# electronicarts/mesh2splat

Measured on AMD Instinct MI355X. Metric: Gaussians/sec emitted (mesh->3DGS conversion pass, density 1024^2), higher is better.
Workload: dtype f32

## Files before the change

mesh2splat_amd/csrc/m2s_devfn.h:

```cpp
#pragma once
#include "m2s_device.h"
#include "m2s_exact.h"

#pragma clang fp contract(off)

namespace m2s {

__device__ __forceinline__ float len3(float x, float y, float z) { return sqrtf((x * x + y * y) + z * z); }
__device__ __forceinline__ float len3sq(float x, float y, float z) { return (x * x + y * y) + z * z; }
__device__ __forceinline__ float inv_len3(float x, float y, float z) {
    const float q = len3sq(x, y, z);
    if (wave_all(in_sqrt_range(q))) return rcp_rn(sqrt_rn(q));
    return 1.0f / sqrtf(q);
}

__device__ __forceinline__ uint32_t wave_incl_scan(uint32_t v, int ) {
    v += (uint32_t)__builtin_amdgcn_update_dpp(0, (int)v, 0x111, 0xf, 0xf, true);
    v += (uint32_t)__builtin_amdgcn_update_dpp(0, (int)v, 0x112, 0xf, 0xf, true);
    v += (uint32_t)__builtin_amdgcn_update_dpp(0, (int)v, 0x114, 0xf, 0xf, true);
    v += (uint32_t)__builtin_amdgcn_update_dpp(0, (int)v, 0x118, 0xf, 0xf, true);
    v += (uint32_t)__builtin_amdgcn_update_dpp(0, (int)v, 0x142, 0xa, 0xf, true);
    v += (uint32_t)__builtin_amdgcn_update_dpp(0, (int)v, 0x143, 0xc, 0xf, true);
    return v;
}
// ... 515 lines not shown
    const uint32_t m = q[2u * (t0 >> 3)], end = q[2u * (t0 >> 3) + 1u];
    uniform = end > t_last;
    return m;
}

__device__ __forceinline__ bool setup_raster_for(const SceneDev& sc, uint32_t t, uint32_t mesh_hint, bool uniform_mesh,
                                                 uint32_t R, Raster& rs) {
    float p[9];
    load_positions(sc.tri, t, p);
    uint32_t m = uniform_mesh ? mesh_hint : find_mesh(sc, sc.tri_first + t);
    const MeshParams* mp = sc.meshes + m;
    Geo g;
    geo_setup(p, mp->bmin, mp->bmax, g);
    return raster_setup(g, R, rs);
}

constexpr float kUnorm8 = 0.003921568859368563f;

struct __attribute__((packed, aligned(4))) ComboPair { uint32_t v[6]; };

typedef const __attribute__((address_space(1))) char* GlobalBytes;
__device__ __forceinline__ GlobalBytes as_global(const void* p) { return (GlobalBytes)p; }
__device__ __forceinline__ ComboPair ld_combo(GlobalBytes base, uint32_t dword_off) {
    const __attribute__((address_space(1))) uint32_t* p = reinterpret_cast<const __attribute__((address_space(1))) uint32_t*>(base + (size_t)(dword_off * 4u));
    ComboPair r;
#pragma unroll
    for (int i = 0; i < 6; ++i) r.v[i] = p[i];
    return r;
}
__device__ __forceinline__ uint32_t ld_texel(GlobalBytes base, uint32_t texel) {
    return *reinterpret_cast<const __attribute__((address_space(1))) uint32_t*>(base + (size_t)(texel * 4u));
}


struct TriShade {
    int a1, b1, a2, b2;
    long long e1, e2;
    float inva, sx, sy, lod0;
    float4 rot;
    float lod1, lod2;
    uint32_t org;
    uint32_t mesh;
};
static_assert(sizeof(TriShade) == 80, "TriShade must be five float4");

struct TriShadeS {
    short a1, b1, a2, b2;
    int e1, e2;
    float inva, sx, sy, lod0;
    float4 rot;
    float lod1, lod2;
    uint32_t org;
    uint32_t mesh;
};
static_assert(sizeof(TriShadeS) == 64, "TriShadeS must be four float4");

__device__ __forceinline__ float lod_from_grad(float fw, float fh, float dudx, float dvdx, float dudy, float dvdy) {
    const float sx = dudx * fw, tx = dvdx * fh, sy = dudy * fw, ty = dvdy * fh;
    const float r2 = fmaxf(fma_(tx, tx, sx * sx), fma_(ty, ty, sy * sy));
    return 0.5f * fast_log2(r2);
}

template <class MP, class TS>
__device__ __forceinline__ void tri_shade_rest(const float p[9], const Geo& g, int a1, int b1, int a2, int b2, MP mp,
                                               float4 b0, float2 b1uv, TS& ts) {
    ts.mesh = 0;
    const float A1 = (float)a1 * 256.0f * ts.inva, B1 = (float)b1 * 256.0f * ts.inva;
    const float A2 = (float)a2 * 256.0f * ts.inva, B2 = (float)b2 * 256.0f * ts.inva;
    geo_flat(p, g, ts.sx, ts.sy, ts.rot);
    ts.lod0 = ts.lod1 = ts.lod2 = 0.0f;
    const auto ta = &mp->tex[0];
    const auto tn = &mp->tex[1];
    const auto tm = &mp->tex[2];
    const bool hasA = ta->texels != nullptr, hasN = tn->texels != nullptr, hasM = tm->texels != nullptr;
    if (hasA || hasN || hasM) {
        const float du1 = b0.z - b0.x, du2 = b1uv.x - b0.x, dv1 = b0.w - b0.y, dv2 = b1uv.y - b0.y;
        const float dudx = fma_(A2, du2, A1 * du1), dvdx = fma_(A2, dv2, A1 * dv1);
        const float dudy = fma_(B2, du2, B1 * du1), dvdy = fma_(B2, dv2, B1 * dv1);
        if (hasA) ts.lod0 = lod_from_grad((float)ta->w, (float)ta->h, dudx, dvdx, dudy, dvdy);
        if (hasN) ts.lod1 = (hasA && tn->w == ta->w && tn->h == ta->h) ? ts.lod0
                          : lod_from_grad((float)tn->w, (float)tn->h, dudx, dvdx, dudy, dvdy);
        if (hasM) ts.lod2 = (hasA && tm->w == ta->w && tm->h == ta->h) ? ts.lod0
                          : (hasN && tm->w == tn->w && tm->h == tn->h) ? ts.lod1
                          : lod_from_grad((float)tm->w, (float)tm->h, dudx, dvdx, dudy, dvdy);
        if (mp->combo.texels != nullptr) {
            const uint32_t nl = ta->n_levels;
            const float q = (float)(nl - 1), lambda = ts.lod0;
            float d = 0.0f, f = 0.0f;
            if (lambda > 0.0f) {
                if (lambda >= q) d = q;
                else { d = floorf(lambda); f = lambda - d; }
            }
            const uint32_t l0 = (uint32_t)d, l1 = min(l0 + 1u, nl - 1u);
            const uint32_t c1 = mp->combo.coff[1], c2 = mp->combo.coff[2], c3 = mp->combo.coff[3], c4 = mp->combo.coff[4];
            const uint32_t off0 = l0 == 0 ? 0u : l0 == 1 ? c1 : l0 == 2 ? c2 : l0 == 3 ? c3 : c4;
            const uint32_t off1 = l1 == 0 ? 0u : l1 == 1 ? c1 : l1 == 2 ? c2 : l1 == 3 ? c3 : c4;
            ts.lod0 = f;
            ts.lod1 = __uint_as_float(off0);
            ts.lod2 = __uint_as_float(off1);
            ts.mesh = (l0 | (l1 << 4)) << 24;
        }
    }
}

template <class MP>
__device__ __forceinline__ void tri_shade_setup(const float p[9], const Geo& g, const Raster& rs, MP mp,
                                                float4 b0, float2 b1, TriShade& ts) {
    {
#pragma clang fp contract(off)
        ts.inva = rcp_rn((float)rs.area2);
    }
    const long long Px0 = 256ll * rs.x0 + 128, Py0 = 256ll * rs.y0 + 128;
    ts.a1 = rs.a[1]; ts.b1 = rs.b[1]; ts.a2 = rs.a[2]; ts.b2 = rs.b[2];
    ts.e1 = (long long)rs.a[1] * Px0 + (long long)rs.b[1] * Py0 + rs.c[1];
    ts.e2 = (long long)rs.a[2] * Px0 + (long long)rs.b[2] * Py0 + rs.c[2];
    ts.org = ((uint32_t)rs.y0 << 12) | (uint32_t)rs.x0;
    tri_shade_rest(p, g, rs.a[1], rs.b[1], rs.a[2], rs.b[2], mp, b0, b1, ts);
}

template <class MP>
__device__ __forceinline__ void tri_shade_small(const float p[9], const Geo& g, const RasterHead& h, const RasterSmall& rs, MP mp, float4 b0, float2 b1,
                                                uint32_t m, TriShadeS& c) {
    {
#pragma clang fp contract(off)
        c.inva = rcp_rn((float)rs.area2);
    }
    c.a1 = (short)rs.a[1]; c.b1 = (short)rs.b[1]; c.a2 = (short)rs.a[2]; c.b2 = (short)rs.b[2];
    c.e1 = rs.e[1]; c.e2 = rs.e[2];
    c.org = ((uint32_t)h.y0 << 12) | (uint32_t)h.x0;
    tri_shade_rest(p, g, rs.a[1], rs.b[1], rs.a[2], rs.b[2], mp, b0, b1, c);
    c.mesh |= m;
}

struct TexTap {
    uint32_t o00, o10, o01, o11;
    float w00, w10, w01, w11;
};

__device__ __forceinline__ void tex_tap(uint32_t W, uint32_t H, uint32_t level_off, float uf, float vf, TexTap& t) {
    float up, vp;
    {
#pragma clang fp contract(off)
        up = uf * (float)W - 0.5f;
        vp = vf * (float)H - 0.5f;
    }
    const float fi = floorf(up), fj = floorf(vp);
    const float a = up - fi, b = vp - fj;
    int i0 = (int)fi, j0 = (int)fj;
    int i1 = i0 + 1, j1 = j0 + 1;
    i0 = i0 < 0 ? i0 + (int)W : i0;
    j0 = j0 < 0 ? j0 + (int)H : j0;
    i1 = i1 >= (int)W ? i1 - (int)W : i1;
    j1 = j1 >= (int)H ? j1 - (int)H : j1;
    const uint32_t r0 = level_off + __umul24((uint32_t)j0, W), r1 = level_off + __umul24((uint32_t)j1, W);
    t.o00 = r0 + (uint32_t)i0; t.o10 = r0 + (uint32_t)i1;
    t.o01 = r1 + (uint32_t)i0; t.o11 = r1 + (uint32_t)i1;
    const float na = 1.0f - a, nb = 1.0f - b;
    t.w00 = na * nb; t.w10 = a * nb; t.w01 = na * b; t.w11 = a * b;
}

struct TexState {
    TexTap lo, hi;
    float f;
};

template <class TD>
__device__ __forceinline__ void tex_state(TD t, float uf, float vf, float lambda, TexState& st) {
    const uint32_t nl = t->n_levels, w = t->w, h = t->h;
    const float q = (float)(nl - 1);
    float d = 0.0f, f = 0.0f;
    if (lambda > 0.0f) {
        if (lambda >= q) d = q;
        else { d = floorf(lambda); f = lambda - d; }
    }
    const uint32_t l0 = (uint32_t)d, l1 = min(l0 + 1u, nl - 1u);
    const uint32_t o1 = t->off[1], o2 = t->off[2], o3 = t->off[3], o4 = t->off[4];
    const uint32_t off0 = l0 == 0 ? 0u : l0 == 1 ? o1 : l0 == 2 ? o2 : l0 == 3 ? o3 : o4;
    const uint32_t off1 = l1 == 0 ? 0u : l1 == 1 ? o1 : l1 == 2 ? o2 : l1 == 3 ? o3 : o4;
    tex_tap(max(1u, w >> l0), max(1u, h >> l0), off0, uf, vf, st.lo);
    st.f = f;
    if (__ballot(f != 0.0f) != 0ull) tex_tap(max(1u, w >> l1), max(1u, h >> l1), off1, uf, vf, st.hi);
    else st.hi = st.lo;
}

struct TexFetch { uint32_t lo[4], hi[4]; };
__device__ __forceinline__ void tex_issue(const uint32_t* __restrict__ texels, const TexState& st, TexFetch& tf) {
    const GlobalBytes gb = as_global(texels);
    tf.lo[0] = ld_texel(gb, st.lo.o00); tf.lo[1] = ld_texel(gb, st.lo.o10); tf.lo[2] = ld_texel(gb, st.lo.o01); tf.lo[3] = ld_texel(gb, st.lo.o11);
    tf.hi[0] = ld_texel(gb, st.hi.o00); tf.hi[1] = ld_texel(gb, st.hi.o10); tf.hi[2] = ld_texel(gb, st.hi.o01); tf.hi[3] = ld_texel(gb, st.hi.o11);
}
template <int NCH>
__device__ __forceinline__ void tap_filter(const uint32_t t[4], const TexTap& tp, float out[NCH]) {
#pragma unroll
    for (int ch = 0; ch < NCH; ch++) {
        const float c00 = (float)((t[0] >> (8 * ch)) & 255u), c10 = (float)((t[1] >> (8 * ch)) & 255u);
        const float c01 = (float)((t[2] >> (8 * ch)) & 255u), c11 = (float)((t[3] >> (8 * ch)) & 255u);
        out[ch] = fma_(tp.w11, c11, fma_(tp.w01, c01, fma_(tp.w10, c10, tp.w00 * c00)));
    }
}
template <int NCH>
__device__ __forceinline__ void tex_finish(const TexFetch& tf, const TexState& st, float out[NCH]) {
    float lo[NCH], hi[NCH];
    tap_filter<NCH>(tf.lo, st.lo, lo);
    tap_filter<NCH>(tf.hi, st.hi, hi);
    const float f = st.f, nf = 1.0f - st.f;
#pragma unroll
    for (int ch = 0; ch < NCH; ch++) out[ch] = fma_(f, hi[ch], nf * lo[ch]) * kUnorm8;
}


struct ComboTap {
    uint32_t o0, o1;
    float w00, w10, w01, w11;
};

__device__ __forceinline__ void combo_tap(uint32_t level_off, uint32_t W, uint32_t H, float uf, float vf, ComboTap& t) {
    float up, vp;
    {
#pragma clang fp contract(off)
        up = uf * (float)W - 0.5f;
        vp = vf * (float)H - 0.5f;
    }
    const float fi = floorf(up), fj = floorf(vp);
    const float a = up - fi, b = vp - fj;
    int i0 = (int)fi, j0 = (int)fj;
    int j1 = j0 + 1;
    i0 = i0 < 0 ? i0 + (int)W : i0;
    j0 = j0 < 0 ? j0 + (int)H : j0;
    j1 = j1 >= (int)H ? j1 - (int)H : j1;
    const uint32_t stride = W + 1;
    t.o0 = level_off + (__umul24((uint32_t)j0, stride) + (uint32_t)i0) * 3u;
    t.o1 = level_off + (__umul24((uint32_t)j1, stride) + (uint32_t)i0) * 3u;
    const float na = 1.0f - a, nb = 1.0f - b;
    t.w00 = na * nb; t.w10 = a * nb; t.w01 = na * b; t.w11 = a * b;
}

__device__ __forceinline__ void combo_filter(const ComboPair& r0, const ComboPair& r1, const ComboTap& t, float out[9]) {
#define M2S_CH(word, sh) fma_(t.w11, (float)((r1.v[(word) + 3] >> (sh)) & 255u), fma_(t.w01, (float)((r1.v[word] >> (sh)) & 255u), \
                          fma_(t.w10, (float)((r0.v[(word) + 3] >> (sh)) & 255u), t.w00 * (float)((r0.v[word] >> (sh)) & 255u))))
    out[0] = M2S_CH(0, 0); out[1] = M2S_CH(0, 8); out[2] = M2S_CH(0, 16); out[3] = M2S_CH(0, 24);
    out[4] = M2S_CH(1, 0); out[5] = M2S_CH(1, 8); out[6] = M2S_CH(1, 16);
    out[7] = M2S_CH(2, 8); out[8] = M2S_CH(2, 16);
#undef M2S_CH
}

__device__ __forceinline__ float frac_repeat(float u) {
    float f = u - floorf(u);
    f = (f >= 0.0f) ? f : 0.0f;
    return fminf(f, 1.0f);
}

struct ComboFetch {
    ComboTap tlo, thi;
    ComboPair a0, a1, b0, b1;
    float f;
};
template <class MP, class TD, class TS>
__device__ __forceinline__ void combo_issue(MP mp, TD t, float uf, float vf, const TS& ts, ComboFetch& cf) {
    const uint32_t w = t->w, h = t->h;
    const float f = ts.lod0;
    const uint32_t off0 = __float_as_uint(ts.lod1), off1 = __float_as_uint(ts.lod2);
    const uint32_t l0 = (ts.mesh >> 24) & 15u, l1 = ts.mesh >> 28;
    const uint32_t* __restrict__ base = mp->combo.texels;
    ComboTap& tlo = cf.tlo;
    ComboTap& thi = cf.thi;
    cf.f = f;
    combo_tap(off0, max(1u, w >> l0), max(1u, h >> l0), uf, vf, tlo);
    combo_tap(off1, max(1u, w >> l1), max(1u, h >> l1), uf, vf, thi);
    const GlobalBytes gb = as_global(base);
    cf.a0 = ld_combo(gb, tlo.o0);
    cf.a1 = ld_combo(gb, tlo.o1);
    cf.b0 = ld_combo(gb, thi.o0);
    cf.b1 = ld_combo(gb, thi.o1);
#ifdef M2S_FUSED3_PRIO
    __builtin_amdgcn_s_setprio(0);
#endif
}
__device__ __forceinline__ void combo_finish(ComboFetch& cf, float out[9]) {
    ComboTap& tlo = cf.tlo;
    ComboTap& thi = cf.thi;
    const float f = cf.f;
    const float klo = (1.0f - f) * kUnorm8, khi = f * kUnorm8;
    tlo.w00 *= klo; tlo.w10 *= klo; tlo.w01 *= klo; tlo.w11 *= klo;
    thi.w00 *= khi; thi.w10 *= khi; thi.w01 *= khi; thi.w11 *= khi;
    float lo[9], hi[9];
    combo_filter(cf.a0, cf.a1, tlo, lo);
    combo_filter(cf.b0, cf.b1, thi, hi);
#pragma unroll
    for (int ch = 0; ch < 9; ch++) out[ch] = lo[ch] + hi[ch];
}
template <class MP, class TD, class TS>
__device__ __forceinline__ void combo_sample(MP mp, TD t, float uf, float vf, const TS& ts, float out[9]) {
    ComboFetch cf;
    combo_issue(mp, t, uf, vf, ts, cf);
    combo_finish(cf, out);
}


template <typename T>
__device__ __forceinline__ T ld_plane(const T* base, uint32_t t) {
    return *reinterpret_cast<const T*>(reinterpret_cast<const char*>(base) + (size_t)(t * (uint32_t)sizeof(T)));
}


template <class MP, class TS = TriShade, bool kComboOnly = false>
__device__ __forceinline__ void shade_from_tri(const TriPlanes& tp, uint32_t t, int x, int y, MP mp,
                                               const TS& ts, float4 rec[6], unsigned long long* stamps = nullptr,
                                               const float2* uvl = nullptr ) {
    const int dx256 = (x - (int)(ts.org & 0xFFFu)) * 256, dy256 = (y - (int)(ts.org >> 12)) * 256;
    float l1, l2;
    if constexpr (sizeof(ts.e1) == 4) {
        const int E1 = ts.e1 + (int)ts.a1 * dx256 + (int)ts.b1 * dy256;
        const int E2 = ts.e2 + (int)ts.a2 * dx256 + (int)ts.b2 * dy256;
        l1 = (float)E1 * ts.inva;
        l2 = (float)E2 * ts.inva;
    } else {
        const long long E1 = ts.e1 + (long long)ts.a1 * dx256 + (long long)ts.b1 * dy256;
        const long long E2 = ts.e2 + (long long)ts.a2 * dx256 + (long long)ts.b2 * dy256;
        l1 = i64_to_f32(E1) * ts.inva;
        l2 = i64_to_f32(E2) * ts.inva;
    }

    float4 b0 = make_float4(0, 0, 0, 0);
    float2 b1 = make_float2(0, 0);
    if (uvl == nullptr) {
        b0 = ld_plane(tp.B0, t);
        b1 = ld_plane(tp.B1, t);
    }
    const float4 a0 = ld_plane(tp.A0, t), a1 = ld_plane(tp.A1, t);
    const float a2 = ld_plane(tp.A2, t);
    const float4 c0 = ld_plane(tp.C0, t), c1 = ld_plane(tp.C1, t);
    const float c2 = ld_plane(tp.C2, t);
    const float4 d0 = ld_plane(tp.D0, t), d1 = ld_plane(tp.D1, t), d2 = ld_plane(tp.D2, t);
    float U, V;
    {
#pragma clang fp contract(off)
        if (uvl != nullptr) {
            const float2 q0 = uvl[0], q1 = uvl[1], q2 = uvl[2];
            U = (q0.x + l1 * q1.x) + l2 * q2.x;
            V = (q0.y + l1 * q1.y) + l2 * q2.y;
        } else {
            U = (b0.x + l1 * (b0.z - b0.x)) + l2 * (b1.x - b0.x);
            V = (b0.y + l1 * (b0.w - b0.y)) + l2 * (b1.y - b0.y);
        }
    }
#define M2S_LERP(f0, f1, f2) fma_(l2, (f2) - (f0), fma_(l1, (f1) - (f0), (f0)))

    const auto ta = &mp->tex[0];
    const auto tn = &mp->tex[1];
    const auto tm = &mp->tex[2];
    const uint32_t* xa = ta->texels;
    const uint32_t* xn = tn->texels;
    const uint32_t* xm = tm->texels;
    if (stamps) stamps[0] = __builtin_amdgcn_s_memtime();
    const float uf = frac_repeat(U), vf = frac_repeat(V);
    float col[4] = { 1.0f, 1.0f, 1.0f, 1.0f };
    float nrm[3] = { 0.0f, 0.0f, 1.0f };
    float metal = 0.1f, rough = 0.5f;
    const uint32_t* __restrict__ cmb = mp->combo.texels;
    if (cmb != nullptr) {
        float acc[9];
        combo_sample(mp, ta, uf, vf, ts, acc);
        col[0] = acc[0]; col[1] = acc[1]; col[2] = acc[2]; col[3] = acc[3];
        nrm[0] = acc[4]; nrm[1] = acc[5]; nrm[2] = acc[6];
        rough = acc[7]; metal = acc[8];
    } else if constexpr (!kComboOnly) {
        TexState sa, sn, sm;
        TexFetch fa, fn, fm;
        const bool n_like_a = xa != nullptr && xn != nullptr && tn->w == ta->w && tn->h == ta->h;
        const bool m_like_a = xa != nullptr && xm != nullptr && tm->w == ta->w && tm->h == ta->h;
        const bool m_like_n = xn != nullptr && xm != nullptr && tm->w == tn->w && tm->h == tn->h;
        if (xa != nullptr) tex_state(ta, uf, vf, ts.lod0, sa);
        if (xn != nullptr) { if (n_like_a) sn = sa; else tex_state(tn, uf, vf, ts.lod1, sn); }
        if (xm != nullptr) {
            if (xn != nullptr ? m_like_n : m_like_a) sm = (xn != nullptr) ? sn : sa;
            else tex_state(tm, uf, vf, ts.lod2, sm);
        }
        if (xa != nullptr) tex_issue(xa, sa, fa);
        if (xn != nullptr) tex_issue(xn, sn, fn);
        if (xm != nullptr) tex_issue(xm, sm, fm);
        if (xa != nullptr) tex_finish<4>(fa, sa, col);
        if (xn != nullptr) tex_finish<3>(fn, sn, nrm);
        if (xm != nullptr) {
            float sv[3];
            tex_finish<3>(fm, sm, sv);
            metal = sv[2]; rough = sv[1];
        }
    }
    if (stamps) stamps[1] = __builtin_amdgcn_s_memtime();
    const float Pxw = M2S_LERP(a0.x, a0.w, a1.z), Pyw = M2S_LERP(a0.y, a1.x, a1.w), Pzw = M2S_LERP(a0.z, a1.y, a2);
    const float Nx = M2S_LERP(c0.x, c0.w, c1.z), Ny = M2S_LERP(c0.y, c1.x, c1.w), Nz = M2S_LERP(c0.z, c1.y, c2);
    float ox = Nx, oy = Ny, oz = Nz;
    if (xn != nullptr) {
        const float Tx = M2S_LERP(d0.x, d1.x, d2.x), Ty = M2S_LERP(d0.y, d1.y, d2.y), Tz = M2S_LERP(d0.z, d1.z, d2.z);
        const float Tw = M2S_LERP(d0.w, d1.w, d2.w);
        float rx = fma_(nrm[0], 2.0f, -1.0f), ry = fma_(nrm[1], 2.0f, -1.0f), rz = fma_(nrm[2], 2.0f, -1.0f);
        float inv = fast_rsq(dot3_(rx, ry, rz, rx, ry, rz));
        rx *= inv; ry *= inv; rz *= inv;
        float bx = fma_(Ny, Tz, -(Nz * Ty)), by = fma_(Nz, Tx, -(Nx * Tz)), bz = fma_(Nx, Ty, -(Ny * Tx));
        inv = fast_rsq(dot3_(bx, by, bz, bx, by, bz)) * Tw;
        bx *= inv; by *= inv; bz *= inv;
        inv = fast_rsq(dot3_(Nx, Ny, Nz, Nx, Ny, Nz));
        const float nnx = Nx * inv, nny = Ny * inv, nnz = Nz * inv;
        const float wx = fma_(nnx, rz, fma_(bx, ry, Tx * rx)), wy = fma_(nny, rz, fma_(by, ry, Ty * rx)), wz = fma_(nnz, rz, fma_(bz, ry, Tz * rx));
        inv = fast_rsq(dot3_(wx, wy, wz, wx, wy, wz));
        ox = wx * inv; oy = wy * inv; oz = wz * inv;
    }
#undef M2S_LERP
    if (stamps) stamps[2] = __builtin_amdgcn_s_memtime();
    rec[0] = make_float4(Pxw, Pyw, Pzw, 1.0f);
    rec[1] = make_float4(col[0] * mp->color[0], col[1] * mp->color[1], col[2] * mp->color[2], col[3] * mp->color[3]);
    rec[2] = make_float4(ts.sx, ts.sy, 1e-7f, 0.0f);
    rec[3] = make_float4(ox, oy, oz, 0.0f);
    rec[4] = ts.rot;
    rec[5] = make_float4(metal, rough, 0.0f, 1.0f);
}

__device__ __forceinline__ void nt_store(float4* p, float4 v) {
    __builtin_nontemporal_store(v.x, &p->x); __builtin_nontemporal_store(v.y, &p->y);
    __builtin_nontemporal_store(v.z, &p->z); __builtin_nontemporal_store(v.w, &p->w);
}

}
```

mesh2splat_amd/csrc/m2s_fused3.hip:

```cpp
#include "m2s_fused_common.h"

#pragma clang fp contract(off)

namespace m2s {

#ifndef M2S_FUSED3_WAVES
#define M2S_FUSED3_WAVES 4
#endif
#ifndef M2S_FUSED3_ENTRIES
#define M2S_FUSED3_ENTRIES 1024
#endif
#ifndef M2S_FUSED3_STAGE
#define M2S_FUSED3_STAGE (M2S_FUSED3_WAVES >= 5 ? 16 : 32)
#endif
constexpr int kL3Team = 4;
constexpr int kL3Threads = kL3Team * 64;
constexpr uint32_t kL3Entries = (uint32_t)M2S_FUSED3_ENTRIES * kL3Team;
constexpr int kL3Stage = M2S_FUSED3_STAGE;
constexpr uint32_t kL3Wait = 1u << 24;
constexpr uint32_t kL3Stop = 1u << 28;

struct F3Ctl {
    unsigned long long base;
    unsigned long long total_w[kL3Team];
    uint32_t total_c[kL3Team];
    uint32_t counted[kL3Team];
    uint32_t expanded[kL3Team];
    uint32_t t0[kL3Team];
    uint32_t claimed;
    uint32_t base_state;
    uint32_t flags;
    uint32_t pad_;
};
struct F3Lds {
    float4 tri[kL3Team][64 * 4];
    uint32_t tskip[kL3Team][64];
    uint16_t entries[kL3Entries];
    float4 stage[kL3Team][kL3Stage * 6];
    F3Ctl ctl;
};
static_assert(sizeof(F3Lds) * M2S_FUSED3_WAVES <= 163840, "M2S_FUSED3_WAVES workgroups per CU must fit the 160 KB of LDS");
constexpr uint32_t kF3Irregular = 1u << 8;

__device__ __forceinline__ uint32_t l3_load(const uint32_t* p) { return __hip_atomic_load(p, __ATOMIC_ACQUIRE, __HIP_MEMORY_SCOPE_WORKGROUP); }
__device__ __forceinline__ void l3_store(uint32_t* p, uint32_t v) { __hip_atomic_store(p, v, __ATOMIC_RELEASE, __HIP_MEMORY_SCOPE_WORKGROUP); }
__device__ __forceinline__ uint32_t l3_uniform(const uint32_t* p) {
    return __builtin_amdgcn_readfirstlane(__hip_atomic_load(p, __ATOMIC_RELAXED, __HIP_MEMORY_SCOPE_WORKGROUP));
}
__device__ __forceinline__ void l3_fail(F3Ctl& C, uint32_t why, int lane) {
    if (lane == 0) {
        __hip_atomic_fetch_or(&C.flags, why, __ATOMIC_RELEASE, __HIP_MEMORY_SCOPE_WORKGROUP);
        __hip_atomic_fetch_add(&C.claimed, kL3Stop, __ATOMIC_RELAXED, __HIP_MEMORY_SCOPE_WORKGROUP);
    }
}

__device__ __forceinline__ bool f3_get_base(F3Ctl& C, unsigned long long* chain, uint32_t b0, int lane, uint32_t epoch, uint32_t* status,
                                            unsigned long long& base) {
    uint32_t st = l3_load(&C.base_state);
    if (st != 2) {
        uint32_t got = 1;
        if (lane == 0) {
            uint32_t expect = 0;
            got = __hip_atomic_compare_exchange_strong(&C.base_state, &expect, 1u, __ATOMIC_ACQ_REL, __ATOMIC_ACQUIRE, __HIP_MEMORY_SCOPE_WORKGROUP) ? 0u : 1u;
        }
        got = __builtin_amdgcn_readfirstlane(got);
        if (got == 0) {
            const unsigned long long b = b0 == 0 ? 0ull : lookback(chain, b0, lane, epoch, status);
            if (lane == 0) {
                C.base = b;
                chain_store(&chain[b0], kFlagPrefix | ((unsigned long long)epoch << kEpochShift) | ((b + C.total_w[0]) & kValMask));
            }
            l3_store(&C.base_state, 2u);
        } else {
            uint32_t spins = 0;
            while (l3_load(&C.base_state) != 2) {
                if (++spins > kL3Wait) { l3_fail(C, 1u, lane); return false; }
                __builtin_amdgcn_s_sleep(2);
            }
        }
    }
    base = C.base;
    return true;
}

#ifdef M2S_TIMELINE
__device__ unsigned long long g_tl_f3[16384 * 4 * 8];
#define TLF(k) do { __builtin_amdgcn_sched_barrier(0); if (lane == 0 && blockIdx.x < 16384u) g_tl_f3[((size_t)blockIdx.x * 4 + wave) * 8 + (k)] = wall_clock64(); __builtin_amdgcn_sched_barrier(0); } while (0)
#define TLFV(k, v) do { if (lane == 0 && blockIdx.x < 16384u) g_tl_f3[((size_t)blockIdx.x * 4 + wave) * 8 + (k)] = (v); } while (0)
#else
#define TLF(k) do { } while (0)
#define TLFV(k, v) do { } while (0)
#endif

__global__ void __launch_bounds__(kL3Threads, M2S_FUSED3_WAVES) k_fused3(SceneDev sc, uint32_t R, unsigned long long* __restrict__ chain,
                                                      unsigned long long limit, float4* __restrict__ out,
                                                      unsigned long long* __restrict__ total_out,
                                                      uint32_t* __restrict__ status , uint32_t epoch,
                                                      BigItem* __restrict__ biglist, uint32_t* __restrict__ bigmeta,
                                                      uint32_t tpw ,
                                                      RunInfo runs, BatchTable bt) {
    __shared__ F3Lds S;
    F3Ctl& C = S.ctl;
    const int lane = threadIdx.x & 63;
    const uint32_t wave = __builtin_amdgcn_readfirstlane(threadIdx.x >> 6);
    const uint32_t n_batches = bt.first ? bt.n : (sc.n_tri + tpw - 1u) / tpw;
    const uint32_t hb = blockIdx.x, xcd = hb & 7u, round = hb >> 3;
    const bool in_runs = runs.base != nullptr;
    const uint32_t rmask = (1u << runs.shift) - 1u;
    const unsigned long long etag = (unsigned long long)epoch << kEpochShift;
    uint32_t lb = hb;
    if (in_runs) {
        uint32_t rr = ((round >> runs.shift) << 3) + xcd;
        if (runs.order) rr = ((const __attribute__((address_space(4))) uint32_t*)runs.order)[rr];
        lb = (rr << runs.shift) + (round & rmask);
    }
    const bool band_first = in_runs && (round & rmask) == 0u;
    if (lb * (uint32_t)kL3Team >= n_batches) return;
    TLF(0);
    if (lane == 0) { C.counted[wave] = 0; C.expanded[wave] = 0; }
    if (wave == 0 && lane == 0) {
        C.claimed = 0; C.flags = 0;
        C.base_state = (lb == 0 || band_first) ? 2u : 0u;
        C.base = band_first ? runs.base[lb >> runs.shift] : 0ull;
    }
    __syncthreads();
    const uint32_t b0 = lb * kL3Team;
    const uint32_t nb_here = min((uint32_t)kL3Team, n_batches - b0);
    const uint32_t b = b0 + wave;
    const bool has_batch = wave < nb_here;
    const unsigned long long band_base = band_first ? C.base : 0ull;

    uint32_t t0 = b * tpw, nt = tpw;
    if (bt.first && has_batch) {
        const __attribute__((address_space(4))) uint32_t* q = (const __attribute__((address_space(4))) uint32_t*)bt.first;
        t0 = q[b];
        nt = q[b + 1] - t0;
    }
    const uint32_t t = t0 + lane;
    const bool valid = has_batch && (uint32_t)lane < nt && t < sc.n_tri;
    if (lane == 0) C.t0[wave] = t0;
    int kind = kNone;
    unsigned long long mask = 0;
    uint32_t cnt = 0;
    {
        float p[9];
        Geo g;
        RasterHead h;
        h.x0 = h.y0 = 0; h.x1 = h.y1 = -1; h.ext = 0;
        bool box = false;
        uint32_t m = 0;
        float4 uvb0 = make_float4(0, 0, 0, 0);
        float2 uvb1 = make_float2(0, 0);
        bool uniform_mesh = false;
        uint32_t m0 = 0;
        if (has_batch) {
            const uint32_t lastT = min(t0 + nt, sc.n_tri) - 1;
            m0 = mesh_of_range(sc, t0, lastT, uniform_mesh);
            m = m0;
            if (valid) {
                load_positions(sc.tri, t, p);
                uvb0 = sc.tri.B0[t];
                uvb1 = sc.tri.B1[t];
                if (uniform_mesh) geo_setup_mp(p, kConstMesh(sc.meshes + m0), g);
                else { m = find_mesh(sc, sc.tri_first + t); geo_setup_mp(p, sc.meshes + m, g); }
                box = raster_head(g, R, h);
            }
        }
        const int w = h.x1 - h.x0 + 1, rows = h.y1 - h.y0 + 1;
        RasterSmall rs;
        bool small = box && w <= 8 && rows <= 8 && h.ext <= 2304;
        if (small) small = raster_small(h, rs);
        else if (box) kind = kBig;
        {
            uint32_t mlo = 0, mhi = 0;
            small_coverage(small, w, rows, rs, mlo, mhi);
            mask = (unsigned long long)mlo | ((unsigned long long)mhi << 32);
            cnt = (uint32_t)__popc(mlo) + (uint32_t)__popc(mhi);
            if (small) kind = kSmall;
        }
        if (cnt != 0 && kind == kSmall) {
            TriShadeS c;
            if (uniform_mesh) tri_shade_small(p, g, h, rs, kConstMesh(sc.meshes + m0), uvb0, uvb1, m, c);
            else tri_shade_small(p, g, h, rs, sc.meshes + m, uvb0, uvb1, m, c);
            const float4* src = reinterpret_cast<const float4*>(&c);
#pragma unroll
            for (int k = 0; k < 4; ++k) S.tri[wave][lane * 4 + k] = src[k];
        }
        if (__ballot(kind == kBig) != 0ull) {
            Raster rb;
            rb.x0 = rb.y0 = 0; rb.x1 = rb.y1 = -1; rb.ext = 0; rb.bias = 0; rb.area2 = 1;
#pragma unroll
            for (int i = 0; i < 3; i++) { rb.a[i] = rb.b[i] = 0; rb.c[i] = 0; }
            if (kind == kBig && !raster_setup(g, R, rb)) kind = kNone;
            unsigned long long bigm = __ballot(kind == kBig);
            while (bigm) {
                const int src = __ffsll((long long)bigm) - 1;
                bigm &= bigm - 1;
                const Raster br = shfl_raster(rb, src);
                uint32_t part = 0;
                for (int y = br.y0 + lane; y <= br.y1; y += 64) {
                    int xa, xb;
                    row_span(br, y, xa, xb);
                    part += (uint32_t)max(xb - xa + 1, 0);
                }
                part = wave_sum(part);
                if (lane == src) cnt = part;
            }
        }
    }
    if (cnt == 0) kind = kNone;
    const uint32_t cntc = kind == kSmall ? cnt : 0;
    const bool anybig = __ballot(kind == kBig) != 0ull;

    const uint32_t incl = wave_incl_scan(cnt, lane);
    const uint32_t inclc = wave_incl_scan(cntc, lane);
    const unsigned long long total_w = __builtin_amdgcn_readlane(incl, 63);
    const uint32_t total_c = __builtin_amdgcn_readlane(inclc, 63);
    const uint32_t toff = incl - cnt;
    const uint32_t ctoff = inclc - cntc;

    if (has_batch && lane == 0) {
        const bool knows = b == 0 || (band_first && wave == 0);
        chain_store(&chain[b], (knows ? kFlagPrefix : kFlagAgg) | etag | (((knows ? band_base : 0ull) + total_w) & kValMask));
    }
    if (lane == 0) {
        C.total_w[wave] = total_w; C.total_c[wave] = total_c;
        if (anybig) __hip_atomic_fetch_or(&C.flags, kF3Irregular, __ATOMIC_RELAXED, __HIP_MEMORY_SCOPE_WORKGROUP);
    }
    l3_store(&C.counted[wave], 1u);
    TLF(1);

    uint32_t stream0 = 0;
    unsigned long long out0 = 0;
    bool alive = true;
    for (uint32_t k = 0; k < wave && alive; ++k) {
        uint32_t spins = 0;
        while (l3_load(&C.counted[k]) == 0) {
            if (++spins > kL3Wait) { alive = false; break; }
            __builtin_amdgcn_s_sleep(1);
        }
        stream0 += C.total_c[k];
        out0 += C.total_w[k];
    }
    if (!alive) l3_fail(C, 1u, lane);
    if (alive && (unsigned long long)stream0 + total_c > kL3Entries) {
        alive = false;
        l3_fail(C, 2u, lane);
    }
    unsigned long long base = 0;
    bool have_base = false;
    if (alive && wave == (uint32_t)kL3Team - 1 && (l3_load(&C.flags) & 0xFFu) == 0) {
        have_base = f3_get_base(C, chain, b0, lane, epoch, status, base);
        if (!have_base) alive = false;
    }

    if (alive) {
        if (cntc) S.tskip[wave][lane] = (uint32_t)((out0 + toff) - ((unsigned long long)stream0 + ctoff));
        if (anybig) {
            unsigned long long bb;
            if (f3_get_base(C, chain, b0, lane, epoch, status, bb)) {
                if (kind == kBig) {
                    const uint32_t slot = atomicAdd(&bigmeta[0], 1u);
                    atomicMax(&bigmeta[1], cnt);
                    atomicAdd(&bigmeta[2], cnt);
                    BigItem it2;
                    it2.t = t; it2.cnt = cnt; it2.off = bb + out0 + toff;
                    biglist[slot] = it2;
                }
                if (lane == 0) __hip_atomic_store(&status[0], 1u, __ATOMIC_RELAXED, __HIP_MEMORY_SCOPE_SYSTEM);
            } else alive = false;
        }
        if (kind == kSmall) {
            unsigned long long mm = mask;
            uint32_t ci = stream0 + ctoff;
            const uint32_t tag = (uint32_t)lane << 6;
            while (mm) {
                const int bit = __ffsll((long long)mm) - 1;
                mm &= mm - 1;
                S.entries[ci++] = (uint16_t)(tag | (uint32_t)bit);
            }
        }
    }
    l3_store(&C.expanded[wave], 1u);
    TLF(2);
    [[maybe_unused]] unsigned long long tl_strips = 0;

    for (uint32_t k = 0; k < (uint32_t)kL3Team && alive; ++k) {
        uint32_t spins = 0;
        while (l3_load(&C.counted[k]) == 0) {
            if (++spins > kL3Wait) { alive = false; l3_fail(C, 1u, lane); break; }
            __builtin_amdgcn_s_sleep(1);
        }
    }
    float4* const stage = S.stage[wave];
    uint32_t exp_seen = 0;
    TLF(3);
    while (alive) {
        uint32_t s = 0;
        if (lane == 0) s = __hip_atomic_fetch_add(&C.claimed, 1u, __ATOMIC_RELAXED, __HIP_MEMORY_SCOPE_WORKGROUP);
        s = __builtin_amdgcn_readfirstlane(s);
        const uint32_t c1 = l3_uniform(&C.total_c[0]), c2 = c1 + l3_uniform(&C.total_c[1]), c3 = c2 + l3_uniform(&C.total_c[2]),
                       stream_total = c3 + l3_uniform(&C.total_c[3]);
        const uint32_t pos0 = s * 64u;
        if (s >= kL3Stop / 64u || pos0 >= stream_total) break;
#ifdef M2S_TIMELINE
        ++tl_strips;
#endif
        const uint32_t n = min(64u, stream_total - pos0);
        if (exp_seen != 15u) {
            const uint32_t lo[4] = { 0u, c1, c2, c3 }, hi[4] = { c1, c2, c3, stream_total };
#pragma unroll
            for (int k = 0; k < kL3Team; ++k) {
                if ((exp_seen >> k) & 1u) continue;
                if (hi[k] <= pos0 || lo[k] >= pos0 + n) continue;
                uint32_t spins = 0;
                while (l3_load(&C.expanded[k]) == 0) {
                    if (++spins > kL3Wait) { alive = false; l3_fail(C, 1u, lane); break; }
                    __builtin_amdgcn_s_sleep(1);
                }
                exp_seen |= 1u << k;
            }
            if (!alive) break;
        }
#ifdef M2S_FUSED3_PRIO
        __builtin_amdgcn_s_setprio(M2S_FUSED3_PRIO);
#endif
        const uint32_t pos = pos0 + (uint32_t)lane;
        const bool have = (uint32_t)lane < n;
        uint32_t en = 0;
        if (have) en = S.entries[pos];
        const uint32_t ow = (pos >= c1 ? 1u : 0u) + (pos >= c2 ? 1u : 0u) + (pos >= c3 ? 1u : 0u);
        const uint32_t tl = (en >> 6) & 63u, bit = en & 63u;
        float4 rec[6];
        uint32_t my_mesh = 0;
        if (have) my_mesh = reinterpret_cast<const uint32_t*>(&S.tri[ow][tl * 4 + 3])[3] & 0xFFFFFFu;
        unsigned long long todo = __ballot(have);
        while (todo) {
            const uint32_t m_now = __builtin_amdgcn_readlane(my_mesh, __ffsll((long long)todo) - 1);
            const bool mine = have && my_mesh == m_now;
            if (mine) {
                const TriShadeS& ts = *reinterpret_cast<const TriShadeS*>(&S.tri[ow][tl * 4]);
                const uint32_t tt = C.t0[ow] + tl;
                const uint32_t org = ts.org;
                const int x = (int)(org & 0xFFFu) + (int)(bit & 7u), y = (int)(org >> 12) + (int)(bit >> 3);
                shade_from_tri<ConstMeshPtr, TriShadeS, true>(sc.tri, tt, x, y, kConstMesh(sc.meshes + __builtin_amdgcn_readfirstlane(my_mesh)), ts, rec);
            }
            todo &= ~__ballot(mine);
        }
        if (!have_base) {
            if (!f3_get_base(C, chain, b0, lane, epoch, status, base)) break;
            have_base = true;
        }
        const uint32_t fl = l3_load(&C.flags);
        if (fl & 0xFFu) break;
        const unsigned long long base_now = (unsigned long long)l3_uniform(reinterpret_cast<const uint32_t*>(&C.base)) |
                                            ((unsigned long long)l3_uniform(reinterpret_cast<const uint32_t*>(&C.base) + 1) << 32);
        if ((fl & kF3Irregular) == 0) {
            const unsigned long long o0 = base_now + pos0;
            uint32_t nvalid = n;
            if (o0 + 64ull > limit) {
                if (o0 >= limit) nvalid = 0;
                else if (limit - o0 < nvalid) nvalid = (uint32_t)(limit - o0);
            }
#pragma unroll 1
            for (int part = 0; part < 64 / kL3Stage; ++part) {
                if (have && (lane / kL3Stage) == part) {
#pragma unroll
                    for (int k = 0; k < 6; ++k) stage[(lane % kL3Stage) * 6 + k] = rec[k];
                }
                wave_lds_sync();
                float4* __restrict__ dsto = out + (o0 + (uint32_t)kL3Stage * part) * 6;
                const uint32_t nv = nvalid > (uint32_t)kL3Stage * part ? min((uint32_t)kL3Stage, nvalid - (uint32_t)kL3Stage * part) : 0u;
#pragma unroll
                for (int j = 0; j < (kL3Stage * 6 + 63) / 64; ++j) {
                    const uint32_t q = (uint32_t)lane + 64u * j;
                    const uint32_t r = q / 6u;
                    if (r < nv) nt_store(&dsto[q], stage[q]);
                }
                wave_lds_sync();
            }
        } else if (have) {
            const unsigned long long oidx = base_now + S.tskip[ow][tl] + pos;
            if (oidx < limit) {
                float4* __restrict__ dsto = out + oidx * 6;
#pragma unroll
                for (int k = 0; k < 6; ++k) nt_store(&dsto[k], rec[k]);
            }
        }
    }
    TLF(4);
    TLFV(6, tl_strips);
    const uint32_t err = l3_load(&C.flags) & 0xFFu;
    if (alive && wave == nb_here - 1 && err == 0) {
        if (!have_base) have_base = f3_get_base(C, chain, b0, lane, epoch, status, base);
        if (have_base && lane == 0) {
            const unsigned long long out_total = (C.total_w[0] + C.total_w[1]) + (C.total_w[2] + C.total_w[3]);
            chain_store(&chain[b0 + nb_here - 1], kFlagPrefix | etag | ((base + out_total) & kValMask));
            if (b0 + nb_here == n_batches) *total_out = base + out_total;
            if (runs.out && (lb & rmask) == 0u) runs.out[lb >> runs.shift] = base;
        }
    }
    if (err && lane == 0) __hip_atomic_store(&status[1], err, __ATOMIC_RELAXED, __HIP_MEMORY_SCOPE_SYSTEM);
    TLF(5);
    TLFV(7, (unsigned long long)lb);
}

void launch_fused3(const SceneDev& sc, uint32_t R, unsigned long long* chain, uint64_t limit, float4* out,
                   unsigned long long* total, uint32_t* status, uint32_t epoch, BigItem* biglist, uint32_t* bigmeta,
                   const RunInfo& runs, const BatchTable& bt, hipStream_t st) {
    const uint32_t tpw = fused_tpw(sc.n_tri);
    const uint32_t n_batches = bt.first ? bt.n : n_fused_waves(sc.n_tri);
    if (!n_batches) return;
    uint32_t nb = (n_batches + kL3Team - 1) / kL3Team;
    RunInfo r = runs;
    if (tpw != 64u || bt.first) r = RunInfo{ nullptr, nullptr, 0u, nullptr };
    if (r.base) r.out = nullptr;
    if (r.base) nb = ((nb + (8u << r.shift) - 1u) / (8u << r.shift)) * (8u << r.shift);
    else nb = (nb + 7u) & ~7u;
    hipLaunchKernelGGL(k_fused3, dim3(nb), dim3(kL3Threads), 0, st, sc, R, chain, (unsigned long long)limit, out, total, status,
                       epoch & 0xFFFFu, biglist, bigmeta, tpw, r, bt);
}

#ifdef M2S_TIMELINE
}
extern "C" int m2s_debug_timeline_f3(void* dst, size_t bytes) {
    return hipMemcpyFromSymbol(dst, HIP_SYMBOL(m2s::g_tl_f3), std::min(bytes, sizeof(m2s::g_tl_f3))) == hipSuccess ? 0 : 1;
}
extern "C" int m2s_debug_timeline_f3_clear() {
    void* p = nullptr;
    if (hipGetSymbolAddress(&p, HIP_SYMBOL(m2s::g_tl_f3)) != hipSuccess) return 1;
    return hipMemset(p, 0, sizeof(m2s::g_tl_f3)) == hipSuccess ? 0 : 2;
}
namespace m2s {
#endif
hipError_t preload_fused3() { hipFuncAttributes a; return hipFuncGetAttributes(&a, reinterpret_cast<const void*>(&k_fused3)); }

}
```

Baseline: 26.17 billion.

## Shrink LDS pixel entries to bytes and cache per-triangle UVs in LDS

Pixel entries in LDS shrink from 16-bit to 8-bit. The owning triangle is no longer stored per entry; it is recovered through a per-wave cumulative-count table and a lane map using ballot/mbcnt. Per-triangle UV bases and deltas are now kept in LDS, so shading reads them locally instead of loading the B0/B1 planes from global memory. Optional macros add nontemporal attribute loads and LDS-sourced positions. The aim is lower LDS footprint and fewer global loads, paid for with extra ballot/popcount work per strip.

```diff
diff --git a/mesh2splat_amd/csrc/m2s_devfn.h b/mesh2splat_amd/csrc/m2s_devfn.h
--- a/mesh2splat_amd/csrc/m2s_devfn.h
+++ b/mesh2splat_amd/csrc/m2s_devfn.h
@@ -841,11 +841,24 @@
     return *reinterpret_cast<const T*>(reinterpret_cast<const char*>(base) + (size_t)(t * (uint32_t)sizeof(T)));
 }
 
-
-template <class MP, class TS = TriShade, bool kComboOnly = false>
+template <bool kNT, typename T>
+__device__ __forceinline__ T ld_attr(const T* base, uint32_t t) {
+    if constexpr (!kNT) return ld_plane(base, t);
+    else {
+        const T* p = reinterpret_cast<const T*>(reinterpret_cast<const char*>(base) + (size_t)(t * (uint32_t)sizeof(T)));
+        if constexpr (sizeof(T) == 16) {
+            return make_float4(__builtin_nontemporal_load(&p->x), __builtin_nontemporal_load(&p->y),
+                               __builtin_nontemporal_load(&p->z), __builtin_nontemporal_load(&p->w));
+        } else return __builtin_nontemporal_load(p);
+    }
+}
+
+
+template <class MP, class TS = TriShade, bool kComboOnly = false, bool kStreamAttr = false>
 __device__ __forceinline__ void shade_from_tri(const TriPlanes& tp, uint32_t t, int x, int y, MP mp,
                                                const TS& ts, float4 rec[6], unsigned long long* stamps = nullptr,
-                                               const float2* uvl = nullptr ) {
+                                               const float2* uvl = nullptr ,
+                                               const float* posl = nullptr ) {
     const int dx256 = (x - (int)(ts.org & 0xFFFu)) * 256, dy256 = (y - (int)(ts.org >> 12)) * 256;
     float l1, l2;
     if constexpr (sizeof(ts.e1) == 4) {
@@ -866,11 +879,20 @@
         b0 = ld_plane(tp.B0, t);
         b1 = ld_plane(tp.B1, t);
     }
-    const float4 a0 = ld_plane(tp.A0, t), a1 = ld_plane(tp.A1, t);
-    const float a2 = ld_plane(tp.A2, t);
-    const float4 c0 = ld_plane(tp.C0, t), c1 = ld_plane(tp.C1, t);
-    const float c2 = ld_plane(tp.C2, t);
-    const float4 d0 = ld_plane(tp.D0, t), d1 = ld_plane(tp.D1, t), d2 = ld_plane(tp.D2, t);
+    float4 a0, a1;
+    float a2;
+    if (posl == nullptr) {
+        a0 = ld_plane(tp.A0, t); a1 = ld_plane(tp.A1, t);
+        a2 = ld_plane(tp.A2, t);
+    }
+    const float4 c0 = ld_attr<kStreamAttr>(tp.C0, t), c1 = ld_attr<kStreamAttr>(tp.C1, t);
+    const float c2 = ld_attr<kStreamAttr>(tp.C2, t);
+    const float4 d0 = ld_attr<kStreamAttr>(tp.D0, t), d1 = ld_attr<kStreamAttr>(tp.D1, t), d2 = ld_attr<kStreamAttr>(tp.D2, t);
+    if (posl != nullptr) {
+        a0 = make_float4(posl[0], posl[1], posl[2], posl[3]);
+        a1 = make_float4(posl[4], posl[5], posl[6], posl[7]);
+        a2 = posl[8];
+    }
     float U, V;
     {
 #pragma clang fp contract(off)
diff --git a/mesh2splat_amd/csrc/m2s_fused3.hip b/mesh2splat_amd/csrc/m2s_fused3.hip
--- a/mesh2splat_amd/csrc/m2s_fused3.hip
+++ b/mesh2splat_amd/csrc/m2s_fused3.hip
@@ -35,11 +35,20 @@
 struct F3Lds {
     float4 tri[kL3Team][64 * 4];
     uint32_t tskip[kL3Team][64];
-    uint16_t entries[kL3Entries];
+    float2 uv[kL3Team][64 * 3];
+    uint16_t cum[kL3Team][64];
+    uint8_t lane_of[kL3Team][64];
+    uint8_t entries[kL3Entries];
     float4 stage[kL3Team][kL3Stage * 6];
     F3Ctl ctl;
 };
 static_assert(sizeof(F3Lds) * M2S_FUSED3_WAVES <= 163840, "M2S_FUSED3_WAVES workgroups per CU must fit the 160 KB of LDS");
+static_assert((uint32_t)M2S_FUSED3_ENTRIES * kL3Team < 0xFFFFu && 64u * 64u < 0xFFFFu, "cum is 16 bits wide, 0xFFFF marks an unused slot");
+#ifdef M2S_FUSED3_NT_ATTR
+constexpr bool kF3StreamAttr = true;
+#else
+constexpr bool kF3StreamAttr = false;
+#endif
 constexpr uint32_t kF3Irregular = 1u << 8;
 
 __device__ __forceinline__ uint32_t l3_load(const uint32_t* p) { return __hip_atomic_load(p, __ATOMIC_ACQUIRE, __HIP_MEMORY_SCOPE_WORKGROUP); }
@@ -185,6 +194,10 @@
             const float4* src = reinterpret_cast<const float4*>(&c);
 #pragma unroll
             for (int k = 0; k < 4; ++k) S.tri[wave][lane * 4 + k] = src[k];
+            float2* const uvs = &S.uv[wave][lane * 3];
+            uvs[0] = make_float2(uvb0.x, uvb0.y);
+            uvs[1] = make_float2(uvb0.z - uvb0.x, uvb0.w - uvb0.y);
+            uvs[2] = make_float2(uvb1.x - uvb0.x, uvb1.y - uvb0.y);
         }
         if (__ballot(kind == kBig) != 0ull) {
             Raster rb;
@@ -256,6 +269,16 @@
 
     if (alive) {
         if (cntc) S.tskip[wave][lane] = (uint32_t)((out0 + toff) - ((unsigned long long)stream0 + ctoff));
+        {
+            const unsigned long long cov = __ballot(cntc != 0);
+            const uint32_t ncov = (uint32_t)__popcll(cov);
+            if ((uint32_t)lane >= ncov) S.cum[wave][lane] = 0xFFFFu;
+            if (cntc) {
+                const uint32_t slot = __builtin_amdgcn_mbcnt_hi((uint32_t)(cov >> 32), __builtin_amdgcn_mbcnt_lo((uint32_t)cov, 0u));
+                S.cum[wave][slot] = (uint16_t)inclc;
+                S.lane_of[wave][slot] = (uint8_t)lane;
+            }
+        }
         if (anybig) {
             unsigned long long bb;
             if (f3_get_base(C, chain, b0, lane, epoch, status, bb)) {
@@ -273,11 +296,12 @@
         if (kind == kSmall) {
             unsigned long long mm = mask;
             uint32_t ci = stream0 + ctoff;
-            const uint32_t tag = (uint32_t)lane << 6;
+            uint32_t first = 64u;
             while (mm) {
                 const int bit = __ffsll((long long)mm) - 1;
                 mm &= mm - 1;
-                S.entries[ci++] = (uint16_t)(tag | (uint32_t)bit);
+                S.entries[ci++] = (uint8_t)(first | (uint32_t)bit);
+                first = 0u;
             }
         }
     }
@@ -307,8 +331,8 @@
         ++tl_strips;
 #endif
         const uint32_t n = min(64u, stream_total - pos0);
+        const uint32_t lo[4] = { 0u, c1, c2, c3 }, hi[4] = { c1, c2, c3, stream_total };
         if (exp_seen != 15u) {
-            const uint32_t lo[4] = { 0u, c1, c2, c3 }, hi[4] = { c1, c2, c3, stream_total };
 #pragma unroll
             for (int k = 0; k < kL3Team; ++k) {
                 if ((exp_seen >> k) & 1u) continue;
@@ -330,7 +354,23 @@
         uint32_t en = 0;
         if (have) en = S.entries[pos];
         const uint32_t ow = (pos >= c1 ? 1u : 0u) + (pos >= c2 ? 1u : 0u) + (pos >= c3 ? 1u : 0u);
-        const uint32_t tl = (en >> 6) & 63u, bit = en & 63u;
+        const uint32_t bit = en & 63u;
+        uint32_t slot = 0;
+        {
+            const unsigned long long fm = __ballot(have && (en & 64u) != 0u);
+#pragma unroll
+            for (int k = 0; k < kL3Team; ++k) {
+                if (hi[k] <= pos0 || lo[k] >= pos0 + n || hi[k] == lo[k]) continue;
+                const uint32_t p0 = max(pos0, lo[k]);
+                const uint32_t q0 = p0 - lo[k], sl = p0 - pos0;
+                const uint32_t s0 = (uint32_t)__popcll(__ballot((uint32_t)S.cum[k][lane] <= q0));
+                const unsigned long long fk = fm & ~((2ull << sl) - 1ull);
+                const uint32_t below = __builtin_amdgcn_mbcnt_hi((uint32_t)(fk >> 32), __builtin_amdgcn_mbcnt_lo((uint32_t)fk, 0u));
+                if (ow == (uint32_t)k) slot = s0 + below + (uint32_t)((fk >> lane) & 1ull);
+            }
+        }
+        uint32_t tl = 0;
+        if (have) tl = S.lane_of[ow][slot & 63u] & 63u;
         float4 rec[6];
         uint32_t my_mesh = 0;
         if (have) my_mesh = reinterpret_cast<const uint32_t*>(&S.tri[ow][tl * 4 + 3])[3] & 0xFFFFFFu;
@@ -343,7 +383,18 @@
                 const uint32_t tt = C.t0[ow] + tl;
                 const uint32_t org = ts.org;
                 const int x = (int)(org & 0xFFFu) + (int)(bit & 7u), y = (int)(org >> 12) + (int)(bit >> 3);
-                shade_from_tri<ConstMeshPtr, TriShadeS, true>(sc.tri, tt, x, y, kConstMesh(sc.meshes + __builtin_amdgcn_readfirstlane(my_mesh)), ts, rec);
+#ifdef M2S_FUSED3_UV_GLOBAL
+                const float2* const uvl = nullptr;
+#else
+                const float2* const uvl = &S.uv[ow][tl * 3];
+#endif
+#ifdef M2S_FUSED3_ABL_POS
+                const float* const posl = reinterpret_cast<const float*>(&S.tri[ow][tl * 4]);
+#else
+                const float* const posl = nullptr;
+#endif
+                shade_from_tri<ConstMeshPtr, TriShadeS, true, kF3StreamAttr>(sc.tri, tt, x, y, kConstMesh(sc.meshes + __builtin_amdgcn_readfirstlane(my_mesh)),
+                                                                              ts, rec, nullptr, uvl, posl);
             }
             todo &= ~__ballot(mine);
         }
```

Result: faster. 26.77 billion, median of 6 (+2.3%).
